# sxyu/plenoctree

Measured on AMD Instinct MI355X. Metric: training rays/sec (800x800, 64+128 samples), higher is better.
Workload: dtype f32

## Files before the change

plenoctree_amd/csrc/mlp_kernels.hip:

```cpp
#include "pxo_mlp.h"

namespace pxo {

__global__ void pack_fwd_kernel(const float* __restrict__ p, int deg, float* __restrict__ out) {
  const int nhb = head_blocks(deg);
  const int64_t total = fwd_image_floats(deg);
  const int64_t bias_off = fwd_bias_off(deg);
  for (int64_t idx = blockIdx.x * (int64_t)blockDim.x + threadIdx.x; idx < total;
       idx += (int64_t)gridDim.x * blockDim.x) {
    float v;
    if (idx >= bias_off) {
      v = fwd_image_bias(p, deg, (int)(idx - bias_off));
    } else {
      int l = 0;
      while (l < 8 && idx >= fwd_layer_off(l + 1)) ++l;
      int64_t loc = idx - fwd_layer_off(l);
      const int ncb = l < 8 ? 8 : nhb;
      int j = (int)(loc & 3), lane = (int)((loc >> 2) & 63);
      int64_t cg = loc >> 8;
      int c = (int)(cg % ncb), g = (int)(cg / ncb);
      int k = 8 * g + 4 * (lane >> 5) + j, n = 32 * c + (lane & 31);
      v = src_weight(p, deg, l, k, n);
    }
    out[idx] = v;
  }
}

__global__ void pack_bwd_kernel(const float* __restrict__ p, int deg, float* __restrict__ out) {
  const int nhb = head_blocks(deg);
  const int64_t total = bwd_image_floats(deg);
  const int64_t head_sz = (int64_t)nhb * 32 * 256;
  for (int64_t idx = blockIdx.x * (int64_t)blockDim.x + threadIdx.x; idx < total;
       idx += (int64_t)gridDim.x * blockDim.x) {
    int l;
    int64_t loc;
    if (idx < head_sz) { l = 8; loc = idx; }
    else { int q = (int)((idx - head_sz) / (256 * 256)); l = 7 - q; loc = idx - head_sz - (int64_t)q * 256 * 256; }
    int j = (int)(loc & 3), lane = (int)((loc >> 2) & 63);
    int64_t cg = loc >> 8;
    int c = (int)(cg % 8), g = (int)(cg / 8);
    int k = 8 * g + 4 * (lane >> 5) + j, n = 32 * c + (lane & 31);
    out[idx] = src_weight(p, deg, l, n, k);
  }
}

int launch_pack(const PxoCfg* cfg, const float* mlp_params, float* fwd, float* bwd, hipStream_t s) {
  if (cfg->mlp_precision == PXO_MLP_BF16X6) return launch_pack_x6(cfg, mlp_params, fwd, bwd, s);
  if (cfg->mlp_precision == PXO_MLP_BF16X3) {
    if (bwd) { set_error("pack_weights: mlp_precision bf16x3 is forward-only (packed_bwd must be NULL)"); return PXO_ERR_UNSUPPORTED; }
    return launch_pack_x3(cfg, mlp_params, fwd, s);
  }
  hipLaunchKernelGGL(pack_fwd_kernel, dim3(512), dim3(256), 0, s, mlp_params, cfg->sh_deg, fwd);
  if (bwd) hipLaunchKernelGGL(pack_bwd_kernel, dim3(512), dim3(256), 0, s, mlp_params, cfg->sh_deg, bwd);
  return check_launch("pack_weights");
}

__global__ void posenc_kernel(const float* __restrict__ x, int64_t N, float* __restrict__ enc) {
  int64_t idx = blockIdx.x * (int64_t)blockDim.x + threadIdx.x;
  if (idx >= N * kEnc) return;
  int64_t r = idx / kEnc;
  int col = (int)(idx - r * kEnc);
  enc[idx] = enc_value(x[r * 3], x[r * 3 + 1], x[r * 3 + 2], col);
}

int launch_posenc(const float* x, int64_t N, float* enc, hipStream_t s) {
  if (N == 0) return PXO_OK;
  int64_t total = N * kEnc;
  hipLaunchKernelGGL(posenc_kernel, dim3((unsigned)((total + 255) / 256)), dim3(256), 0, s, x, N, enc);
  return check_launch("posenc");
}

template <int RBN> struct EncGeom {
  static constexpr int kRows = 32 * RBN;
  static constexpr int kParts = kMlpThreads / kRows;
  static constexpr int kColsPer = kEncPad / kParts;
};
template <int RBN, bool GRID = true, bool KEEP = false>
__device__ __forceinline__ void posenc_tile(float* __restrict__ lds, const float* __restrict__ pts,
                                            const GridSpec& grid, int64_t row0, int64_t M, int tid,
                                            float (*keep)[EncGeom<RBN>::kColsPer] = nullptr) {
  constexpr int kRows = EncGeom<RBN>::kRows, kColsPer = EncGeom<RBN>::kColsPer;
  const int row = tid % kRows, part = tid / kRows;
  const int64_t grow = row0 + row;
  float p0 = 0.f, p1 = 0.f, p2 = 0.f;
  if (grow < M) {
    if (GRID && grid.enabled) grid_point(grid, grow, p0, p1, p2);
    else { p0 = pts[grow * 3]; p1 = pts[grow * 3 + 1]; p2 = pts[grow * 3 + 2]; }
  }
#pragma unroll 4
  for (int i = 0; i < kColsPer; ++i) {
    const int col = part * kColsPer + i;
    const float e = enc_value(p0, p1, p2, col);
    lds[row * kLDA + col] = e;
    if (KEEP) (*keep)[i] = e;
  }
}
template <int RBN>
__device__ __forceinline__ void posenc_restore(float* __restrict__ lds, int tid, const float (&keep)[EncGeom<RBN>::kColsPer]) {
  constexpr int kRows = EncGeom<RBN>::kRows, kColsPer = EncGeom<RBN>::kColsPer;
  const int row = tid % kRows, part = tid / kRows;
#pragma unroll
  for (int i = 0; i < kColsPer; ++i) lds[row * kLDA + part * kColsPer + i] = keep[i];
}

template <int RBN, int CBN>
__device__ __forceinline__ void mfma_group(const f32x4 (&a)[RBN], const f32x4 (&b)[CBN], f32x16 (&acc)[RBN][CBN]) {
#pragma unroll
  for (int j = 0; j < 4; ++j)
#pragma unroll
    for (int r = 0; r < RBN; ++r)
#pragma unroll
      for (int c = 0; c < CBN; ++c)
        acc[r][c] = __builtin_amdgcn_mfma_f32_32x32x2f32(a[r][j], b[c][j], acc[r][c], 0, 0, 0);
}

struct ARows {
  const float* base;
  uint32_t lo, hi;
};
__device__ __forceinline__ ARows make_arows(const float* lds, int lane) {
  ARows a{lds, (uint32_t)((lane & 31) * kLDA + (lane >> 5) * 4), 0u};
  a.hi = a.lo + 2 * 32 * kLDA;
  asm volatile("" : "+v"(a.hi));
  return a;
}
template <int RBN>
__device__ __forceinline__ void load_a(const ARows& ar, int g, f32x4 (&a)[RBN]) {
#pragma unroll
  for (int r = 0; r < RBN; ++r)
    a[r] = *reinterpret_cast<const f32x4*>(ar.base + (r < 2 ? ar.lo : ar.hi) + (r & 1) * 32 * kLDA + g * 8);
}
struct WImage {
  __amdgpu_buffer_rsrc_t rsrc;
  uint32_t voff;
};
__device__ __forceinline__ WImage make_wimage(const float* image, int64_t floats, int lane) {
  return WImage{__builtin_amdgcn_make_buffer_rsrc(const_cast<float*>(image), 0, (int)(floats * 4), 0x00020000),
                (uint32_t)lane * 16u};
}
typedef unsigned int u32x4 __attribute__((ext_vector_type(4)));
template <int CBN>
__device__ __forceinline__ void load_b(const WImage& w, int wu, int g, int kg_stride, f32x4 (&b)[CBN]) {
#pragma unroll
  for (int c = 0; c < CBN; ++c)
    b[c] = __builtin_bit_cast(f32x4, __builtin_amdgcn_raw_buffer_load_b128(w.rsrc, w.voff, (wu + g * kg_stride + c * 64) * 16, 0));
}

constexpr int kBDist = 3;
template <int CBN>
__device__ __forceinline__ void gemm_prefetch_b(const WImage& w, int wu, int kgroups, int kg_stride,
                                                f32x4 (&b)[4][CBN]) {
  const int last = kgroups - 1;
#pragma unroll
  for (int i = 0; i < kBDist; ++i) load_b<CBN>(w, wu, i < last ? i : last, kg_stride, b[i]);
}

struct TileCopy {
  __amdgpu_buffer_rsrc_t out;
  uint32_t voff;
  const float* src;
  uint32_t src_hi;
  bool on;
};
template <int RBN>
__device__ __forceinline__ TileCopy make_tile_copy(const float* lds, float* dst, int64_t row0, int64_t M, int wave, int lane,
                                                   bool on) {
  const int c4 = lane & 7, rsub = lane >> 3;
  const int64_t rows = M - row0 < 32 * RBN ? M - row0 : 32 * RBN;
  TileCopy t;
  t.out = __builtin_amdgcn_make_buffer_rsrc(dst + row0 * kW, 0, on ? (int)(rows * kW * 4) : 0, 0x00020000);
  t.voff = (uint32_t)(rsub * kW + wave * 32 + c4 * 4) * 4u;
  t.src = lds + rsub * kLDA + wave * 32 + c4 * 4;
  t.src_hi = 8 * 8 * kLDA;
  asm volatile("" : "+v"(t.src_hi));
  t.on = on;
  return t;
}
template <int RBN>
__device__ __forceinline__ void tile_copy_slab(const TileCopy& t, int i) {
  const f32x4 v = i < 8 ? *reinterpret_cast<const f32x4*>(t.src + i * 8 * kLDA)
                        : *reinterpret_cast<const f32x4*>(t.src + t.src_hi + (i - 8) * 8 * kLDA);
  __builtin_amdgcn_raw_buffer_store_b128(__builtin_bit_cast(u32x4, v), t.out, t.voff, i * 8 * kW * 4, 0);
}

template <int RBN, int CBN, bool COPY = false>
__device__ __forceinline__ void gemm_lds_packed(const ARows& arow, const WImage& w, int wu,
                                                int kgroups, int kg_stride, f32x16 (&acc)[RBN][CBN],
                                                f32x4 (&b)[4][CBN], const TileCopy* tc = nullptr) {
  constexpr int D = kBDist;
  static_assert(D == 2 || D == 3, "kBDist");
  f32x4 a0[RBN], a1[RBN];
  const int last = kgroups - 1;
  auto cl = [&](int g) { return g < last ? g : last; };
  load_a<RBN>(arow, 0, a0);
  for (int g = 0; g < kgroups; g += 4) {
    load_a<RBN>(arow, g + 1, a1);
    load_b<CBN>(w, wu, cl(g + D), kg_stride, b[D & 3]);
    PXO_PIN();
    mfma_group<RBN, CBN>(a0, b[0], acc);
    PXO_PIN();
    if (COPY && tc->on && g < 4 * RBN) {
      switch (g >> 2) {
        case 0: tile_copy_slab<RBN>(*tc, 0); break;
        case 1: tile_copy_slab<RBN>(*tc, 4 + 0); break;
        case 2: if (RBN > 2) tile_copy_slab<RBN>(*tc, 8 + 0); break;
        default: if (RBN > 2) tile_copy_slab<RBN>(*tc, 12 + 0); break;
      }
      PXO_PIN();
    }
    load_a<RBN>(arow, g + 2, a0);
    load_b<CBN>(w, wu, cl(g + 1 + D), kg_stride, b[(1 + D) & 3]);
    PXO_PIN();
    mfma_group<RBN, CBN>(a1, b[1], acc);
    PXO_PIN();
    if (COPY && tc->on && g < 4 * RBN) {
      switch (g >> 2) {
        case 0: tile_copy_slab<RBN>(*tc, 1); break;
        case 1: tile_copy_slab<RBN>(*tc, 4 + 1); break;
        case 2: if (RBN > 2) tile_copy_slab<RBN>(*tc, 8 + 1); break;
        default: if (RBN > 2) tile_copy_slab<RBN>(*tc, 12 + 1); break;
      }
      PXO_PIN();
    }
    load_a<RBN>(arow, g + 3, a1);
    load_b<CBN>(w, wu, cl(g + 2 + D), kg_stride, b[(2 + D) & 3]);
    PXO_PIN();
    mfma_group<RBN, CBN>(a0, b[2], acc);
    PXO_PIN();
    if (COPY && tc->on && g < 4 * RBN) {
      switch (g >> 2) {
        case 0: tile_copy_slab<RBN>(*tc, 2); break;
        case 1: tile_copy_slab<RBN>(*tc, 4 + 2); break;
        case 2: if (RBN > 2) tile_copy_slab<RBN>(*tc, 8 + 2); break;
        default: if (RBN > 2) tile_copy_slab<RBN>(*tc, 12 + 2); break;
      }
      PXO_PIN();
    }
    load_a<RBN>(arow, cl(g + 4), a0);
    load_b<CBN>(w, wu, cl(g + 3 + D), kg_stride, b[(3 + D) & 3]);
    PXO_PIN();
    mfma_group<RBN, CBN>(a1, b[3], acc);
    PXO_PIN();
    if (COPY && tc->on && g < 4 * RBN) {
      switch (g >> 2) {
        case 0: tile_copy_slab<RBN>(*tc, 3); break;
        case 1: tile_copy_slab<RBN>(*tc, 4 + 3); break;
        case 2: if (RBN > 2) tile_copy_slab<RBN>(*tc, 8 + 3); break;
        default: if (RBN > 2) tile_copy_slab<RBN>(*tc, 12 + 3); break;
      }
      PXO_PIN();
    }
  }
}

template <int CBN>
__device__ __forceinline__ void gemm_head(const float* __restrict__ arow, const f32x4* __restrict__ wp, int cb_stride,
                                          int kg_stride, f32x16 (&acc)[1][CBN]) {
  f32x4 a0[1], a1[1], b0[CBN], b1[CBN], b2[CBN], b3[CBN];
  auto lb = [&](int g, f32x4 (&b)[CBN]) {
#pragma unroll
    for (int c = 0; c < CBN; ++c) b[c] = wp[(int64_t)g * kg_stride + c * cb_stride];
  };
  auto la = [&](int g, f32x4 (&a)[1]) { a[0] = *reinterpret_cast<const f32x4*>(arow + g * 8); };
  lb(0, b0); lb(1, b1);
  la(0, a0);
  for (int g = 0; g < 32; g += 4) {
    la(g + 1, a1); lb(g + 2, b2); PXO_PIN();
    mfma_group<1, CBN>(a0, b0, acc); PXO_PIN();
    la(g + 2, a0); lb(g + 3, b3); PXO_PIN();
    mfma_group<1, CBN>(a1, b1, acc); PXO_PIN();
    la(g + 3, a1); lb(g + 4 < 31 ? g + 4 : 31, b0); PXO_PIN();
    mfma_group<1, CBN>(a0, b2, acc); PXO_PIN();
    la(g + 4 < 31 ? g + 4 : 31, a0); lb(g + 5 < 31 ? g + 5 : 31, b1); PXO_PIN();
    mfma_group<1, CBN>(a1, b3, acc); PXO_PIN();
  }
}

template <int RBN, int CBN>
__device__ __forceinline__ void zero_acc(f32x16 (&acc)[RBN][CBN]) {
#pragma unroll
  for (int r = 0; r < RBN; ++r)
#pragma unroll
    for (int c = 0; c < CBN; ++c)
#pragma unroll
      for (int i = 0; i < 16; ++i) acc[r][c][i] = 0.f;
}

__device__ __forceinline__ int frag_row(int reg, int lane) { return (reg & 3) + 8 * (reg >> 2) + 4 * (lane >> 5); }

template <int RBN>
__device__ __forceinline__ void store_wave_cols(const float* __restrict__ lds, float* __restrict__ dst, int64_t row0,
                                                int64_t M, int wave, int lane) {
  const int c4 = lane & 7, rsub = lane >> 3;
  const int64_t rows = M - row0 < 32 * RBN ? M - row0 : 32 * RBN;
  const __amdgpu_buffer_rsrc_t out = __builtin_amdgcn_make_buffer_rsrc(dst + row0 * kW, 0, (int)(rows * kW * 4), 0x00020000);
  const uint32_t voff = (uint32_t)(rsub * kW + wave * 32 + c4 * 4) * 4u;
  const float* __restrict__ src = lds + rsub * kLDA + wave * 32 + c4 * 4;
#pragma unroll
  for (int i0 = 0; i0 < 4 * RBN; i0 += 4) {
    f32x4 v[4];
#pragma unroll
    for (int i = 0; i < 4; ++i) v[i] = *reinterpret_cast<const f32x4*>(src + (i0 + i) * 8 * kLDA);
#pragma unroll
    for (int i = 0; i < 4; ++i)
      __builtin_amdgcn_raw_buffer_store_b128(__builtin_bit_cast(u32x4, v[i]), out, voff, (i0 + i) * 8 * kW * 4, 0);
  }
}

__device__ __forceinline__ float mask_pop(uint32_t& mw, float x) {
  float r;
  asm volatile("v_add_co_u32 %0, vcc, %0, %0\n\tv_cndmask_b32 %1, 0, %2, vcc" : "+v"(mw), "=v"(r) : "v"(x) : "vcc");
  return r;
}

constexpr int kRB = kTM / 32;
constexpr int kCB = 8 / kMlpWaves;

template <int NHB, bool SAVE, bool RGB, int RBN>
__device__ __forceinline__ void fwd_tile(float* __restrict__ lds, const float* __restrict__ pk,
                                         const float* __restrict__ pts, const GridSpec& grid, int64_t M, int deg,
                                         int64_t row0, int64_t slot, float* __restrict__ raw_rgb,
                                         float* __restrict__ raw_sigma, float* __restrict__ acts,
                                         float* __restrict__ enc_out, uint32_t* __restrict__ mask, int tid, int lane,
                                         int wave) {
  constexpr int kRows = 32 * RBN;
  constexpr int kWordsUsed = RBN * kCB * 16 / 32;
  asm volatile("" : "+v"(tid));
  lane = tid & 63;
  const int C = rgb_channels(deg);
  const float* __restrict__ bias = pk + fwd_bias_off(deg);
  const float* arow1 = lds + (lane & 31) * kLDA + (lane >> 5) * 4;
  const ARows arow = make_arows(lds, lane);
  const WImage wimg = make_wimage(pk, fwd_image_floats(deg), lane);
  const bool full = row0 + kRows <= M;
  lds_barrier();
  float enc_keep[EncGeom<RBN>::kColsPer];
  posenc_tile<RBN, !SAVE, !SAVE>(lds, pts, grid, row0, M, tid, &enc_keep);
  lds_barrier();
  if (SAVE) {
#pragma unroll
    for (int i = 0; i < kRows * kEncPad / 4 / kMlpThreads; ++i) {
      const int idx = tid + kMlpThreads * i;
      const int row = idx >> 4, c4 = idx & 15;
      if (full || row0 + row < M)
        *reinterpret_cast<f32x4*>(enc_out + (row0 + row) * kEncPad + c4 * 4) =
            *reinterpret_cast<const f32x4*>(lds + row * kLDA + c4 * 4);
    }
  }

  f32x16 acc[RBN][kCB];
  f32x4 bfrag[4][kCB];
  auto layer_wp = [&](int l) {
    return (int)(fwd_layer_off(l) / 4) + (wave * kCB) * 64;
  };
  gemm_prefetch_b<kCB>(wimg, layer_wp(0), 8, 8 * 64, bfrag);
  float bl[kCB];
#pragma unroll
  for (int c = 0; c < kCB; ++c) bl[c] = bias[(wave * kCB + c) * 32 + (lane & 31)];
  for (int l = 0; l < kDepth; ++l) {
#pragma unroll
    for (int r = 0; r < RBN; ++r)
#pragma unroll
      for (int c = 0; c < kCB; ++c)
#pragma unroll
        for (int i = 0; i < 16; ++i) acc[r][c][i] = bl[c];
    const int wp = layer_wp(l);
    if (SAVE && l > 0) {
      int lane_c = lane;
      asm volatile("" : "+v"(lane_c));
      const TileCopy tc = make_tile_copy<RBN>(lds, acts + (int64_t)(l - 1) * M * kW, row0, M, wave, lane_c, true);
      gemm_lds_packed<RBN, kCB, true>(arow, wimg, wp, 32, 8 * 64, acc, bfrag, &tc);
    } else {
      gemm_lds_packed<RBN, kCB>(arow, wimg, wp, l == 0 ? 8 : 32, 8 * 64, acc, bfrag);
    }
    if (l == 5) {
      gemm_prefetch_b<kCB>(wimg, wp + 32 * 8 * 64, 8, 8 * 64, bfrag);
      lds_barrier();
      if (SAVE) {
#pragma unroll
        for (int i = 0; i < kRows * kEncPad / 4 / kMlpThreads; ++i) {
          const int idx = tid + kMlpThreads * i;
          const int row = idx >> 4, c4 = idx & 15;
          f32x4 v = {0.f, 0.f, 0.f, 0.f};
          if (full || row0 + row < M) v = *reinterpret_cast<const f32x4*>(enc_out + (row0 + row) * kEncPad + c4 * 4);
          *reinterpret_cast<f32x4*>(lds + row * kLDA + c4 * 4) = v;
        }
      } else {
        posenc_restore<RBN>(lds, tid, enc_keep);
      }
      lds_barrier();
      gemm_lds_packed<RBN, kCB>(arow, wimg, wp + 32 * 8 * 64, 8, 8 * 64, acc, bfrag);
    }
    if (l + 1 < kDepth) {
      gemm_prefetch_b<kCB>(wimg, layer_wp(l + 1), 32, 8 * 64, bfrag);
#pragma unroll
      for (int c = 0; c < kCB; ++c) bl[c] = bias[(l + 1) * kW + (wave * kCB + c) * 32 + (lane & 31)];
    }
    lds_barrier();
    int tid_e = tid;
    asm volatile("" : "+v"(tid_e));
    const int lane_e = tid_e & 63;
    uint32_t mw[kMaskWords];
#pragma unroll
    for (int w = 0; w < kMaskWords; ++w) mw[w] = 0u;
#pragma unroll
    for (int r = 0; r < RBN; ++r)
#pragma unroll
      for (int c = 0; c < kCB; ++c) {
        const int col = (wave * kCB + c) * 32 + (lane_e & 31);
#pragma unroll
        for (int reg = 0; reg < 16; ++reg) {
          const int row = r * 32 + frag_row(reg, lane_e);
          const float v = fmaxf(acc[r][c][reg], 0.f);
          lds[row * kLDA + col] = v;
          if (SAVE) mask_push(mw[((r * kCB + c) * 16 + reg) >> 5], v);
        }
      }
    if (SAVE) {
      uint32_t* mp = mask + ((slot * kDepth + l) * kMlpThreads + tid_e) * kMaskWords;
#pragma unroll
      for (int w = 0; w < kWordsUsed; ++w) mp[w] = mw[w];
      if (l == kDepth - 1) store_wave_cols<RBN>(lds, acts + (int64_t)l * M * kW, row0, M, wave, lane_e);
    }
    lds_barrier();
  }

  {
    constexpr int CSTEP = kMlpWaves / RBN;
    constexpr int HMAX = RGB ? (NHB + CSTEP - 1) / CSTEP : 1;
    const int rb = wave % RBN, cb0 = wave / RBN;
    const float* ar = arow1 + rb * 32 * kLDA;
    const float* hb = bias + 8 * kW;
#pragma unroll 1
    for (int i = 0; i < HMAX; ++i) {
      const int cb = RGB ? cb0 + i * CSTEP : (cb0 == 0 ? NHB - 1 : NHB);
      if (cb >= NHB) continue;
      f32x16 hacc[1][1];
      zero_acc(hacc);
      const f32x4* wp = reinterpret_cast<const f32x4*>(pk + fwd_layer_off(8)) + cb * 64 + lane;
      gemm_head<1>(ar, wp, 0, NHB * 64, hacc);
      const int col = cb * 32 + (lane & 31);
      const float b = hb[col];
      float* __restrict__ dst = nullptr;
      int64_t stride = 0;
      if (col < C) { if (RGB) { dst = raw_rgb + col; stride = C; } }
      else if (col == C) { dst = raw_sigma; stride = 1; }
      if (dst) {
        const int64_t r0 = row0 + rb * 32 + 4 * (lane >> 5);
        if (full) {
#pragma unroll
          for (int reg = 0; reg < 16; ++reg) dst[(r0 + (reg & 3) + 8 * (reg >> 2)) * stride] = hacc[0][0][reg] + b;
        } else {
#pragma unroll
          for (int reg = 0; reg < 16; ++reg) {
            const int64_t grow = r0 + (reg & 3) + 8 * (reg >> 2);
            if (grow < M) dst[grow * stride] = hacc[0][0][reg] + b;
          }
        }
      }
    }
  }
}

template <int NHB, bool SAVE, bool RGB, bool DYN = false>
__global__ __launch_bounds__(kMlpThreads, kMlpWgPerCu * kMlpWaves / 4) void mlp_fwd_kernel(
    const float* __restrict__ pk, const float* __restrict__ pts, GridSpec grid, int64_t M, int deg, TileSched ts,
    float* __restrict__ raw_rgb, float* __restrict__ raw_sigma, float* __restrict__ acts,
    float* __restrict__ enc_out, uint32_t* __restrict__ mask, unsigned int* __restrict__ tile_counter) {
  __shared__ __attribute__((aligned(16))) float lds[kTM * kLDA + (DYN ? 4 : 0)];
  const int tid = threadIdx.x, lane = tid & 63;
  const int wave = __builtin_amdgcn_readfirstlane(tid >> 6);
  if (!DYN) {
    for (int64_t tile = blockIdx.x; tile < ts.n_full; tile += gridDim.x)
      fwd_tile<NHB, SAVE, RGB, kRB>(lds, pk, pts, grid, M, deg, tile * kTM, tile, raw_rgb, raw_sigma, acts, enc_out,
                                    mask, tid, lane, wave);
    for (int64_t h = blockIdx.x; h < ts.n_half; h += gridDim.x)
      fwd_tile<NHB, SAVE, RGB, kRB / 2>(lds, pk, pts, grid, M, deg, ts.half_row0 + h * (kTM / 2), ts.n_full + h,
                                        raw_rgb, raw_sigma, acts, enc_out, mask, tid, lane, wave);
  } else {
    const TileTicket tk{reinterpret_cast<int*>(lds + kTM * kLDA), tile_counter};
    const int64_t n_slots = ts.n_full + ts.n_half;
    for (int64_t slot = blockIdx.x; slot < n_slots;) {
      const int ticket = tk.draw(tid);
      if (slot < ts.n_full)
        fwd_tile<NHB, SAVE, RGB, kRB>(lds, pk, pts, grid, M, deg, slot * kTM, slot, raw_rgb, raw_sigma, acts, enc_out,
                                      mask, tid, lane, wave);
      else
        fwd_tile<NHB, SAVE, RGB, kRB / 2>(lds, pk, pts, grid, M, deg, ts.half_row0 + (slot - ts.n_full) * (kTM / 2), slot,
                                          raw_rgb, raw_sigma, acts, enc_out, mask, tid, lane, wave);
      slot = tk.take(tid, ticket);
    }
  }
}

unsigned mlp_grid(int64_t M) {
  const int64_t tiles = num_tiles(M), cap = kMlpWgPerCu * (int64_t)num_cus();
  return (unsigned)(tiles < cap ? tiles : cap);
}

static int launch_fwd_any(const PxoCfg* cfg, const float* pk, const float* pts, const GridSpec& grid,
                          int64_t M, float* raw_rgb, float* raw_sigma, float* acts, float* enc,
                          uint32_t* mask, unsigned int* tile_counter, hipStream_t s) {
  if (M == 0) return PXO_OK;
  KernelTimer timer(PXO_PROF_MLP_FWD, M, s);
  dim3 grid_dim(mlp_grid(M)), block(kMlpThreads);
  const TileSched ts = tile_sched(M, grid_dim.x);
  head_switch(cfg->sh_deg, [&](auto nhb) {
    constexpr int NHB = decltype(nhb)::value;
    const auto kernel = acts && raw_rgb && tile_counter ? mlp_fwd_kernel<NHB, true, true, true>
                        : acts && raw_rgb               ? mlp_fwd_kernel<NHB, true, true>
                        : acts                          ? mlp_fwd_kernel<NHB, true, false>
                        : raw_rgb                       ? mlp_fwd_kernel<NHB, false, true>
                                                        : mlp_fwd_kernel<NHB, false, false>;
    hipLaunchKernelGGL(kernel, grid_dim, block, 0, s, pk, pts, grid, M, cfg->sh_deg, ts, raw_rgb, raw_sigma, acts, enc, mask,
                       tile_counter);
  });
  return check_launch("mlp_fwd");
}

int launch_mlp_fwd(const PxoCfg* cfg, const float* packed_fwd, const float* pts, int64_t M,
                   float* raw_rgb, float* raw_sigma, float* acts, float* enc, uint32_t* mask,
                   hipStream_t s, unsigned int* tile_counter) {
  if (cfg->mlp_precision == PXO_MLP_BF16X6)
    return launch_mlp_fwd_x6(cfg, packed_fwd, pts, 0, 0, nullptr, nullptr, M, raw_rgb, raw_sigma, acts, enc, mask, tile_counter, s);
  if (cfg->mlp_precision == PXO_MLP_BF16X3) {
    if (acts || enc || mask) { set_error("mlp_fwd: mlp_precision bf16x3 is inference-only (no saved tensors)"); return PXO_ERR_UNSUPPORTED; }
    return launch_mlp_fwd_x3(cfg, packed_fwd, pts, 0, 0, nullptr, nullptr, M, raw_rgb, raw_sigma, s);
  }
  return launch_fwd_any(cfg, packed_fwd, pts, make_grid_spec(false, 0, 0, nullptr, nullptr), M, raw_rgb, raw_sigma, acts, enc,
                        mask, tile_counter, s);
}

int launch_mlp_fwd_grid(const PxoCfg* cfg, const float* packed_fwd, int reso, int x0, int x1,
                        const float* off, const float* scale, float* sigma_out, hipStream_t s) {
  const int64_t M = (int64_t)(x1 - x0) * reso * reso;
  if (cfg->mlp_precision == PXO_MLP_BF16X6)
    return launch_mlp_fwd_x6(cfg, packed_fwd, nullptr, reso, x0, off, scale, M, nullptr, sigma_out, nullptr, nullptr, nullptr,
                             nullptr, s);
  if (cfg->mlp_precision == PXO_MLP_BF16X3)
    return launch_mlp_fwd_x3(cfg, packed_fwd, nullptr, reso, x0, off, scale, M, nullptr, sigma_out, s);
  return launch_fwd_any(cfg, packed_fwd, nullptr, make_grid_spec(true, reso, x0, off, scale), M, nullptr, sigma_out, nullptr,
                        nullptr, nullptr, nullptr, s);
}

template <int NHB, int RBN, bool SKIP>
__device__ __forceinline__ int bwd_tile(float* __restrict__ lds, float* __restrict__ db_slot, uint8_t* __restrict__ tile_live,
                                         const float* __restrict__ pkb, const float* __restrict__ d_raw_rgb,
                                         const float* __restrict__ d_raw_sigma, const uint32_t* __restrict__ mask,
                                         int64_t M, int deg, int64_t row0, int64_t slot, float* __restrict__ dz,
                                         int* __restrict__ nz, uint8_t* __restrict__ chunk_live,
                                         int tid, int lane, int wave, int mask_word0 = 0) {
  constexpr int NH = 32 * NHB;
  constexpr int kRows = 32 * RBN;
  constexpr int kWordsUsed = RBN * kCB * 16 / 32;
  constexpr int kChunks = kRows / kLiveRows;
  const int C = rgb_channels(deg);
  const ARows arow = make_arows(lds, lane);
  const WImage wimg = make_wimage(pkb, bwd_image_floats(deg), lane);
  lds_barrier();
  if (SKIP && tid < kChunks) nz[tid] = 0;
  if (SKIP) lds_barrier();
  for (int idx = tid; idx < kRows * NH; idx += kMlpThreads) {
    const int row = idx / NH, col = idx - row * NH;
    const int64_t grow = row0 + row;
    float v = 0.f;
    if (grow < M) {
      if (col < C) { if (d_raw_rgb) v = d_raw_rgb[grow * C + col]; }
      else if (col == C) v = d_raw_sigma[grow];
    }
    lds[row * kLDA + col] = v;
    if (SKIP && v != 0.f) nz[row / kLiveRows] = 1;
  }
  lds_barrier();
  if (SKIP) {
    int any = 0;
#pragma unroll
    for (int c = 0; c < kChunks; ++c) any |= nz[c];
    if (tid < kChunks) chunk_live[row0 / kLiveRows + tid] = (uint8_t)nz[tid];
    if (tid == 0) *tile_live = (uint8_t)(any != 0);
    if (!any) return 0;
    if (RBN == kRB) {
      int lo = 0, hi = 0;
#pragma unroll
      for (int c = 0; c < kChunks / 2; ++c) { lo |= nz[c]; hi |= nz[kChunks / 2 + c]; }
      if (!hi) return 1;
      if (!lo) return 2;
    }
  } else if (tid == 0) {
    *tile_live = 1;
  }
  if (tid < NH) {
    float sum = 0.f;
#pragma unroll 8
    for (int row = 0; row < kRows; ++row) sum += lds[row * kLDA + tid];
    db_slot[8 * kW + tid] = sum;
  }
  if (NH < kW && tid >= NH && tid < kW) db_slot[8 * kW + tid] = 0.f;

  f32x16 acc[RBN][kCB];
  f32x4 bfrag[4][kCB];
  zero_acc(acc);
  uint32_t mw[kMaskWords];
  {
    const uint32_t* mp = mask + ((slot * kDepth + (kDepth - 1)) * kMlpThreads + tid) * kMaskWords + mask_word0;
#pragma unroll
    for (int w = 0; w < kWordsUsed; ++w) mw[w] = mp[w];
    const int wp = (wave * kCB) * 64;
    gemm_prefetch_b<kCB>(wimg, wp, 4 * NHB, 8 * 64, bfrag);
    gemm_lds_packed<RBN, kCB>(arow, wimg, wp, 4 * NHB, 8 * 64, acc, bfrag);
  }
  for (int l = kDepth - 1; l >= 0; --l) {
    const int wp = (int)(bwd_layer_off(l > 0 ? l : 1, deg) / 4) + (wave * kCB) * 64;
    if (l > 0) gemm_prefetch_b<kCB>(wimg, wp, 32, 8 * 64, bfrag);
    lds_barrier();
    int tid_e = tid;
    asm volatile("" : "+v"(tid_e));
    const int lane_e = tid_e & 63;
#pragma unroll
    for (int c = 0; c < kCB; ++c) {
      const int col = (wave * kCB + c) * 32 + (lane_e & 31);
      float colsum = 0.f;
#pragma unroll
      for (int r = 0; r < RBN; ++r)
#pragma unroll
        for (int reg = 0; reg < 16; ++reg) {
          const int row = r * 32 + frag_row(reg, lane_e);
          const float v = mask_pop(mw[((r * kCB + c) * 16 + reg) >> 5], acc[r][c][reg]);
          lds[row * kLDA + col] = v;
          colsum += v;
        }
      colsum += __shfl_xor(colsum, 32);
      if (lane_e < 32) db_slot[l * kW + col] = colsum;
    }
    if (l == 0) store_wave_cols<RBN>(lds, dz, row0, M, wave, lane_e);
    lds_barrier();
    if (l == 0) break;
    zero_acc(acc);
    const uint32_t* mp = mask + ((slot * kDepth + (l - 1)) * kMlpThreads + tid_e) * kMaskWords + mask_word0;
#pragma unroll
    for (int w = 0; w < kWordsUsed; ++w) mw[w] = mp[w];
    const TileCopy tc = make_tile_copy<RBN>(lds, dz + (int64_t)l * M * kW, row0, M, wave, lane, true);
    gemm_lds_packed<RBN, kCB, true>(arow, wimg, wp, 32, 8 * 64, acc, bfrag, &tc);
  }
  return 0;
}

template <int NHB, bool SKIP, bool DYN>
__global__ __launch_bounds__(kMlpThreads, kMlpWgPerCu * kMlpWaves / 4) void mlp_bwd_data_kernel(
    const float* __restrict__ pkb, const float* __restrict__ d_raw_rgb,
    const float* __restrict__ d_raw_sigma, const uint32_t* __restrict__ mask, int64_t M, int deg, TileSched ts,
    float* __restrict__ dz, float* __restrict__ dbias_partial, uint8_t* __restrict__ chunk_live,
    unsigned int* __restrict__ tile_counter) {
  __shared__ __attribute__((aligned(16))) float lds[kTM * kLDA + kTM / kLiveRows + 4];
  int* __restrict__ nz = reinterpret_cast<int*>(lds + kTM * kLDA);
  const int tid = threadIdx.x, lane = tid & 63;
  const int wave = __builtin_amdgcn_readfirstlane(tid >> 6);
  uint8_t* const tile_live = reinterpret_cast<uint8_t*>(dbias_partial + mask_slots(M) * 9 * kW);
  const int64_t n_slots = ts.n_full + ts.n_half;
  auto run = [&](int64_t slot) {
    float* db = dbias_partial + slot * 9 * kW;
    if (slot < ts.n_full) {
      const int half = bwd_tile<NHB, kRB, SKIP>(lds, db, tile_live + slot, pkb, d_raw_rgb, d_raw_sigma, mask, M, deg,
                                                slot * kTM, slot, dz, nz, chunk_live, tid, lane, wave);
      if (SKIP && half)
        bwd_tile<NHB, kRB / 2, SKIP>(lds, db, tile_live + slot, pkb, d_raw_rgb, d_raw_sigma, mask, M, deg,
                                     slot * kTM + (half - 1) * (kTM / 2), slot, dz, nz, chunk_live, tid, lane, wave, half - 1);
    } else
      bwd_tile<NHB, kRB / 2, SKIP>(lds, db, tile_live + slot, pkb, d_raw_rgb, d_raw_sigma, mask, M, deg,
                             ts.half_row0 + (slot - ts.n_full) * (kTM / 2), slot, dz, nz, chunk_live, tid, lane, wave);
  };
  if (!DYN) {
    for (int64_t slot = blockIdx.x; slot < ts.n_full; slot += gridDim.x) run(slot);
    for (int64_t h = blockIdx.x; h < ts.n_half; h += gridDim.x) run(ts.n_full + h);
  } else {
    const TileTicket tk{nz + kTM / kLiveRows, tile_counter};
    for (int64_t slot = blockIdx.x; slot < n_slots;) {
      const int ticket = tk.draw(tid);
      run(slot);
      slot = tk.take(tid, ticket);
    }
  }
}

int mlp_bwd_partials(int64_t M) {
  const TileSched ts = tile_sched(M, mlp_grid(M));
  return (int)(ts.n_full + ts.n_half);
}

int launch_mlp_bwd_data(const PxoCfg* cfg, const float* packed_bwd, const float* d_raw_rgb,
                        const float* d_raw_sigma, const uint32_t* mask, int64_t M, float* dz,
                        float* dbias_partial, uint8_t* chunk_live, unsigned int* tile_counter, hipStream_t s,
                        bool bias_from_wgrad) {
  if (M == 0) return PXO_OK;
  if (cfg->mlp_precision == PXO_MLP_BF16X6)
    return launch_mlp_bwd_data_x6(cfg, packed_bwd, d_raw_rgb, d_raw_sigma, mask, M, dz, dbias_partial, chunk_live, tile_counter, s,
                                  !bias_from_wgrad);
  if (cfg->mlp_precision != PXO_MLP_F32) { set_error("mlp_bwd_data: mlp_precision bf16x3 is inference-only"); return PXO_ERR_UNSUPPORTED; }
  KernelTimer timer(PXO_PROF_MLP_BWD_DATA, M, s);
  dim3 grid_dim(mlp_grid(M)), block(kMlpThreads);
  const TileSched ts = tile_sched(M, grid_dim.x);
  head_switch(cfg->sh_deg, [&](auto nhb) {
    constexpr int NHB = decltype(nhb)::value;
    const auto kernel = chunk_live ? (tile_counter ? mlp_bwd_data_kernel<NHB, true, true> : mlp_bwd_data_kernel<NHB, true, false>)
                                   : (tile_counter ? mlp_bwd_data_kernel<NHB, false, true> : mlp_bwd_data_kernel<NHB, false, false>);
    hipLaunchKernelGGL(kernel, grid_dim, block, 0, s, packed_bwd, d_raw_rgb, d_raw_sigma, mask, M, cfg->sh_deg, ts, dz,
                       dbias_partial, chunk_live, tile_counter);
  });
  return check_launch("mlp_bwd_data");
}

}
```

Baseline: 172,500.

## Tune MLP epilogue LDS addressing and vectorize non-skip backward gradient load

Replaces the per-element row computation in forward and backward epilogues with precomputed base offsets (lo/hi) so LDS stores can use immediate offsets, and does ReLU via inline v_max with an explicit s_nop wait for MFMA results. In the non-SKIP backward tile, the strided gradient load loop with divisions is replaced by a register-staged, clamped-row load pattern that issues all global loads before writing LDS. The aim is to cut VALU address arithmetic and load latency in the epilogue; the hand-placed s_nop padding and asm may interfere with compiler scheduling.

```diff
diff --git a/plenoctree_amd/csrc/mlp_kernels.hip b/plenoctree_amd/csrc/mlp_kernels.hip
--- a/plenoctree_amd/csrc/mlp_kernels.hip
+++ b/plenoctree_amd/csrc/mlp_kernels.hip
@@ -286,8 +286,6 @@
       for (int i = 0; i < 16; ++i) acc[r][c][i] = 0.f;
 }
 
-__device__ __forceinline__ int frag_row(int reg, int lane) { return (reg & 3) + 8 * (reg >> 2) + 4 * (lane >> 5); }
-
 template <int RBN>
 __device__ __forceinline__ void store_wave_cols(const float* __restrict__ lds, float* __restrict__ dst, int64_t row0,
                                                 int64_t M, int wave, int lane) {
@@ -311,6 +309,32 @@
   float r;
   asm volatile("v_add_co_u32 %0, vcc, %0, %0\n\tv_cndmask_b32 %1, 0, %2, vcc" : "+v"(mw), "=v"(r) : "v"(x) : "vcc");
   return r;
+}
+
+__device__ __forceinline__ float relu_acc(float x) {
+  float r;
+  asm("v_max_f32 %0, 0, %1" : "=v"(r) : "v"(x));
+  return r;
+}
+template <int RBN, int CBN>
+__device__ __forceinline__ void mfma_results_ready(f32x16 (&acc)[RBN][CBN]) {
+#pragma unroll
+  for (int r = 0; r < RBN; ++r)
+#pragma unroll
+    for (int c = 0; c < CBN; ++c) asm volatile("s_nop 15\n\ts_nop 1" : "+v"(acc[r][c]));
+}
+
+struct EpiRows {
+  uint32_t lo, hi;
+};
+__device__ __forceinline__ EpiRows make_epi_rows(int col, int lane) {
+  EpiRows e{(uint32_t)(4 * (lane >> 5) * kLDA + col), 0u};
+  e.hi = e.lo + 2 * 32 * kLDA;
+  asm volatile("" : "+v"(e.hi));
+  return e;
+}
+__device__ __forceinline__ uint32_t epi_off(const EpiRows& e, int r, int reg) {
+  return (r < 2 ? e.lo : e.hi) + ((r & 1) * 32 + (reg & 3) + 8 * (reg >> 2)) * kLDA;
 }
 
 constexpr int kRB = kTM / 32;
@@ -403,16 +427,16 @@
     uint32_t mw[kMaskWords];
 #pragma unroll
     for (int w = 0; w < kMaskWords; ++w) mw[w] = 0u;
+    mfma_results_ready(acc);
 #pragma unroll
     for (int r = 0; r < RBN; ++r)
 #pragma unroll
       for (int c = 0; c < kCB; ++c) {
-        const int col = (wave * kCB + c) * 32 + (lane_e & 31);
+        const EpiRows er = make_epi_rows((wave * kCB + c) * 32 + (lane_e & 31), lane_e);
 #pragma unroll
         for (int reg = 0; reg < 16; ++reg) {
-          const int row = r * 32 + frag_row(reg, lane_e);
-          const float v = fmaxf(acc[r][c][reg], 0.f);
-          lds[row * kLDA + col] = v;
+          const float v = relu_acc(acc[r][c][reg]);
+          lds[epi_off(er, r, reg)] = v;
           if (SAVE) mask_push(mw[((r * kCB + c) * 16 + reg) >> 5], v);
         }
       }
@@ -560,16 +584,48 @@
   lds_barrier();
   if (SKIP && tid < kChunks) nz[tid] = 0;
   if (SKIP) lds_barrier();
-  for (int idx = tid; idx < kRows * NH; idx += kMlpThreads) {
-    const int row = idx / NH, col = idx - row * NH;
-    const int64_t grow = row0 + row;
-    float v = 0.f;
-    if (grow < M) {
-      if (col < C) { if (d_raw_rgb) v = d_raw_rgb[grow * C + col]; }
-      else if (col == C) v = d_raw_sigma[grow];
-    }
-    lds[row * kLDA + col] = v;
-    if (SKIP && v != 0.f) nz[row / kLiveRows] = 1;
+  if constexpr (SKIP) {
+    for (int idx = tid; idx < kRows * NH; idx += kMlpThreads) {
+      const int row = idx / NH, col = idx - row * NH;
+      const int64_t grow = row0 + row;
+      float v = 0.f;
+      if (grow < M) {
+        if (col < C) { if (d_raw_rgb) v = d_raw_rgb[grow * C + col]; }
+        else if (col == C) v = d_raw_sigma[grow];
+      }
+      lds[row * kLDA + col] = v;
+      if (v != 0.f) nz[row / kLiveRows] = 1;
+    }
+  } else {
+    constexpr int kPer = kRows / (kMlpThreads / 32);
+    const int c = tid & 31, rsub = tid >> 5;
+    const int last = (int)(M - row0 < kRows ? M - row0 : kRows) - 1;
+    float v[NHB][kPer];
+#pragma unroll
+    for (int cb = 0; cb < NHB; ++cb) {
+      const int col = cb * 32 + c;
+      const float* __restrict__ src = nullptr;
+      int stride = 0;
+      if (col < C) { if (d_raw_rgb) { src = d_raw_rgb + row0 * C + col; stride = C; } }
+      else if (col == C) { src = d_raw_sigma + row0; stride = 1; }
+#pragma unroll
+      for (int i = 0; i < kPer; ++i) v[cb][i] = 0.f;
+      if (src) {
+#pragma unroll
+        for (int i = 0; i < kPer; ++i) {
+          const int row = rsub + kLiveRows * i;
+          v[cb][i] = src[(row < last ? row : last) * stride];
+        }
+      }
+    }
+#pragma unroll
+    for (int cb = 0; cb < NHB; ++cb)
+#pragma unroll
+      for (int i = 0; i < kPer; ++i) {
+        const int row = rsub + kLiveRows * i;
+        const float x = row <= last ? v[cb][i] : 0.f;
+        lds[row * kLDA + cb * 32 + c] = x;
+      }
   }
   lds_barrier();
   if (SKIP) {
@@ -619,14 +675,16 @@
 #pragma unroll
     for (int c = 0; c < kCB; ++c) {
       const int col = (wave * kCB + c) * 32 + (lane_e & 31);
+      EpiRows er{};
+      if constexpr (!SKIP) er = make_epi_rows(col, lane_e);
       float colsum = 0.f;
 #pragma unroll
       for (int r = 0; r < RBN; ++r)
 #pragma unroll
         for (int reg = 0; reg < 16; ++reg) {
-          const int row = r * 32 + frag_row(reg, lane_e);
           const float v = mask_pop(mw[((r * kCB + c) * 16 + reg) >> 5], acc[r][c][reg]);
-          lds[row * kLDA + col] = v;
+          if constexpr (SKIP) lds[(r * 32 + (reg & 3) + 8 * (reg >> 2) + 4 * (lane_e >> 5)) * kLDA + col] = v;
+          else lds[epi_off(er, r, reg)] = v;
           colsum += v;
         }
       colsum += __shfl_xor(colsum, 32);
```

New measurement: 175,000, median of 6. 1.01x the previous value.
